# pyani-plus/pyani-plus

Measured on AMD Instinct MI355X. Metric: pairwise genome comparisons/sec (N x N ANI matrix), higher is better.
Workload: dtype u64

## Files before the change

### pyani_plus_amd/csrc/kmer_hash.hip

```cpp
#include <cstdlib>
#include <type_traits>
#include <utility>

#include "pa_internal.h"
#include "murmur_dev.h"

namespace {

using namespace pa_dev;

constexpr int kThreads = 256;
constexpr uint32_t kStageCap = 1024;
constexpr uint32_t kStageCapSecond = 512;

constexpr int pow2_floor(int k) { int c = 1; while (2 * c <= k) c *= 2; return c; }

__device__ __forceinline__ uint32_t find_genome(const uint32_t *__restrict__ genome_blk, uint32_t n, uint32_t blk) {
  uint32_t lo = 0, hi = n;
  while (hi - lo > 1) {
    uint32_t mid = (lo + hi) >> 1;
    if (genome_blk[mid] <= blk) lo = mid; else hi = mid;
  }
  return lo;
}

__device__ __forceinline__ void region_append(const CandSink &s, uint32_t g, uint64_t h) {
  const uint64_t slot = atomicAdd(&s.cursor[g], 1u);
  if (slot < s.region_off[g + 1] - s.region_off[g]) s.cand_hash[s.region_off[g] + slot] = h; else *s.overflow = 1u;
}

__device__ __forceinline__ void append_candidate(const CandSink &s, uint32_t g, uint64_t h) {
  if (s.region_off) {
    region_append(s, g, h);
  } else {
    const unsigned long long slot = atomicAdd(reinterpret_cast<unsigned long long *>(s.count), 1ULL);
    if (slot < s.cap) {
      s.cand_hash[slot] = h;
      s.cand_genome[slot] = g;
    }
  }
}

template <uint32_t Cap>
__device__ __forceinline__ void stage_candidate(const CandSink &s, uint64_t (&s_hash)[Cap], uint32_t (&s_blk)[Cap],
                                                uint32_t &s_n, uint32_t t, uint64_t h) {
  const uint32_t slot = atomicAdd(&s_n, 1u);
  if (slot < Cap) {
    s_hash[slot] = h;
    s_blk[slot] = t;
  } else if (s.region_off) {
    region_append(s, find_genome(s.genome_blk, s.n_genomes, t), h);
  } else {
    const unsigned long long g = atomicAdd(reinterpret_cast<unsigned long long *>(s.count), 1ULL);
    if (g < s.cap) {
      s.cand_hash[g] = h;
      s.cand_genome[g] = find_genome(s.genome_blk, s.n_genomes, t);
    }
  }
}

template <uint32_t Cap>
__device__ __forceinline__ void flush_staged(const CandSink &s, const uint64_t (&s_hash)[Cap], const uint32_t (&s_blk)[Cap],
                                             const uint32_t &s_n, unsigned long long &s_base, uint32_t blk0, uint32_t n_blocks64) {
  const uint32_t tid = threadIdx.x;
  __syncthreads();
  const uint32_t n = min(s_n, Cap);
  if (n == 0) return;
  if (s.region_off) {
    const uint32_t b0 = blk0 + blockIdx.x * kThreads;
    const uint32_t b1 = min(b0 + (uint32_t)kThreads, n_blocks64) - 1u;
    const uint32_t g0 = find_genome(s.genome_blk, s.n_genomes, b0);
    if (s.genome_blk[g0 + 1] > b1) {
      if (tid == 0) s_base = atomicAdd(&s.cursor[g0], n);
      __syncthreads();
      const uint64_t room = s.region_off[g0 + 1] - s.region_off[g0];
      uint64_t *__restrict__ dst = s.cand_hash + s.region_off[g0];
      for (uint32_t i = tid; i < n; i += kThreads) {
        const uint64_t slot = s_base + i;
        if (slot < room) dst[slot] = s_hash[i]; else *s.overflow = 1u;
      }
    } else {
      for (uint32_t i = tid; i < n; i += kThreads)
        region_append(s, find_genome(s.genome_blk, s.n_genomes, s_blk[i]), s_hash[i]);
    }
    return;
  }
  if (tid == 0) s_base = atomicAdd(reinterpret_cast<unsigned long long *>(s.count), (unsigned long long)n);
  __syncthreads();
  const unsigned long long base = s_base;
  for (uint32_t i = tid; i < n; i += kThreads) {
    const unsigned long long g = base + i;
    if (g < s.cap) {
      s.cand_hash[g] = s_hash[i];
      s.cand_genome[g] = find_genome(s.genome_blk, s.n_genomes, s_blk[i]);
    }
  }
}

__device__ __forceinline__ uint32_t rev_groups32(uint32_t x) {
  x = __builtin_bitreverse32(x);
  return ((x >> 1) & 0x55555555u) | ((x & 0x55555555u) << 1);
}

enum WordForm { kArithmetic = 0, kFirstTables = 1, kSecondTables = 2 };
template <int K, WordForm FORM>
__global__ __launch_bounds__(kThreads) void kmer_hash_kernel(
    const uint4 *__restrict__ packed, const uint2 *__restrict__ mask, const uint64_t *__restrict__ dirty, uint32_t n_blocks64,
    const uint32_t *__restrict__ genome_blk, uint32_t n_genomes, uint64_t max_hash,
    uint64_t *__restrict__ cand_hash, uint32_t *__restrict__ cand_genome, uint64_t cap,
    unsigned long long *__restrict__ count, const uint64_t *__restrict__ region_off, uint32_t *__restrict__ cursor,
    uint32_t *__restrict__ overflow, uint32_t blk0) {
  static_assert(K >= 1 && K <= 32, "a k-mer is one 64-bit register pair");
  constexpr uint32_t kCap = FORM == kSecondTables ? kStageCapSecond : kStageCap;
  __shared__ uint64_t s_hash[kCap];
  __shared__ uint32_t s_blk[kCap];
  __shared__ uint32_t s_n;
  __shared__ unsigned long long s_base;
  constexpr int kWords = (K + 7) / 8;
  __shared__ uint64_t s_lo[FORM == kFirstTables ? kWords : 1][256];
  __shared__ uint4 s_w[FORM == kSecondTables ? kWords : 1][256];
  __shared__ uint32_t s_hi[FORM != kArithmetic ? kWords : 1][256];

  const uint32_t tid = threadIdx.x;
  const CandSink sink{cand_hash, cand_genome, cap, reinterpret_cast<uint64_t *>(count), region_off, cursor, overflow, genome_blk, n_genomes};
  const uint32_t max_hi = (uint32_t)(max_hash >> 32);
  const bool take_all = max_hi == 0xffffffffu;
  const uint32_t screen_hi = max_hi + 1u;
  if (tid == 0) s_n = 0;
  if constexpr (FORM == kFirstTables) fill_first_products(s_lo, s_hi, tid, std::integral_constant<int, K>{});
  if constexpr (FORM == kSecondTables) fill_second_products(s_w, s_hi, tid, K);
  __syncthreads();

  const uint32_t t = blk0 + blockIdx.x * kThreads + tid;
  if (t < n_blocks64) {
    const uint4 cur = packed[t];
    uint2 pw = make_uint2(0u, 0u);
    if (t > 0) pw = reinterpret_cast<const uint2 *>(packed)[2 * (uint64_t)t - 1];
    uint32_t d1 = 0u, d2 = 0u;
    const uint32_t wave_blk = __builtin_amdgcn_readfirstlane(t & ~63u);
    const uint64_t dirty_word = dirty[wave_blk >> 6];
    if ((dirty_word >> (t & 63u)) & 1ull) {
      const uint2 m = mask[t];
      uint32_t d0 = t > 0 ? mask[t - 1].y : 0xffffffffu;
      d1 = m.x;
      d2 = m.y;
      int c = 1;
#pragma unroll
      for (; 2 * c <= K; c *= 2) {
        d2 |= alignbit(d2, d1, 32 - c);
        d1 |= alignbit(d1, d0, 32 - c);
        d0 |= d0 << c;
      }
      constexpr int cc = pow2_floor(K);
      constexpr int r = K - cc;
      if constexpr (r > 0) {
        d2 |= alignbit(d2, d1, 32 - r);
        d1 |= alignbit(d1, d0, 32 - r);
      }
    }
    const uint32_t bad[2] = {d1, d2};
    if ((d1 & d2) != 0xffffffffu) {
      constexpr uint64_t kMask = (K == 32) ? ~0ULL : ((1ULL << (2 * K)) - 1);
      constexpr uint32_t kMaskHi = (uint32_t)(kMask >> 32);
      uint32_t fw[8] = {pw.x, pw.y, cur.x, cur.y, cur.z, cur.w, 0u, 0u};
      uint32_t rw[6];
#pragma unroll
      for (int j = 0; j < 6; ++j) rw[j] = ~rev_groups32(fw[5 - j]);
      auto columns = [&](auto base_tag, int i_begin, int i_end) {
        constexpr int kBase = decltype(base_tag)::value;
#pragma unroll 1
        for (int i = i_begin; i < i_end; ++i) {
          constexpr int kOff = 33 - K;
          const uint32_t fo = 2u * (uint32_t)((i + kOff) & 15), ro = 30u - 2u * (uint32_t)i;
          uint32_t A[5], B[5];
#pragma unroll
          for (int j = 0; j < 5; ++j) {
            A[j] = alignbit(fw[kBase + j + 1], fw[kBase + j], fo);
            B[j] = alignbit(rw[j + 1], rw[j], ro);
          }
#pragma unroll
          for (int wi = 0; wi < 4; ++wi) {
            const uint32_t f_lo = A[wi], f_hi = A[wi + 1], r_lo = B[3 - wi], r_hi = B[4 - wi];
          const uint64_t f_lsb = u64_of(f_lo, f_hi) & kMask, r_lsb = u64_of(r_lo, r_hi) & kMask;
          const uint64_t fwd = __builtin_amdgcn_uicmpl(f_lsb, r_lsb, 37 );
          uint32_t clo, chi;
          asm("s_nop 1\n\tv_cndmask_b32_e64 %0, %1, %2, %3" : "=v"(clo) : "v"((uint32_t)r_lsb), "v"((uint32_t)f_lsb), "s"(fwd));
          asm("v_cndmask_b32_e64 %0, %1, %2, %3" : "=v"(chi) : "v"((uint32_t)(r_lsb >> 32)), "v"((uint32_t)(f_lsb >> 32)), "s"(fwd), "v"(clo));
          uint64_t P[4] = {0, 0, 0, 0};
#pragma unroll
          for (int j = 0; j < kWords; ++j) {
            const uint32_t src = j < 2 ? clo : chi;
            if constexpr (FORM == kSecondTables) {
              P[j] = second_product(s_w, s_hi, j, src);
            } else if constexpr (FORM == kFirstTables) {
              P[j] = first_product(s_lo, s_hi, j, src);
            } else {
              const uint32_t glo = (src >> (16 * (j & 1))) & 0xffu, ghi = (src >> (16 * (j & 1) + 8)) & 0xffu;
              const uint64_t word = u64_of(ascii_group(glo, K - 8 * j), ascii_group(ghi, K - 8 * j - 4));
              P[j] = word * ((j & 1) ? kC2 : kC1);
            }
          }
          (void)kMaskHi;
          uint64_t U, V;
          if constexpr (FORM == kSecondTables) murmur3_pre_last_mul_of_seconds<K>(P, U, V); else murmur3_pre_last_mul<K>(P, U, V);
          if (passes_screen(U, V, take_all, screen_hi)) {
            const uint64_t h = last_mul_and_fold(U, V);
            if (h > max_hash || ((bad[wi >> 1] >> (16 * (wi & 1) + i)) & 1u)) continue;
            stage_candidate(sink, s_hash, s_blk, s_n, t, h);
          }
          }
        }
      };
      constexpr int kOff0 = 33 - K, kSplit = (kOff0 & 15) ? 16 - (kOff0 & 15) : 16;
      columns(std::integral_constant<int, (kOff0 >> 4)>{}, 0, kSplit);
      if constexpr (kSplit < 16) columns(std::integral_constant<int, (kOff0 >> 4) + 1>{}, kSplit, 16);
    }
  }
  flush_staged(sink, s_hash, s_blk, s_n, s_base, blk0, n_blocks64);
}

template <int K>
__global__ __launch_bounds__(kThreads) void kmer_hash_wide_kernel(
    const uint4 *__restrict__ packed, const uint2 *__restrict__ mask, const uint64_t *__restrict__ dirty, uint32_t n_blocks64,
    const uint32_t *__restrict__ genome_blk, uint32_t n_genomes, uint64_t max_hash,
    uint64_t *__restrict__ cand_hash, uint32_t *__restrict__ cand_genome, uint64_t cap,
    unsigned long long *__restrict__ count, const uint64_t *__restrict__ region_off, uint32_t *__restrict__ cursor,
    uint32_t *__restrict__ overflow, uint32_t blk0) {
  static_assert(K >= 33 && K <= 64, "k-mers of 65 to 128 bits");
  __shared__ uint64_t s_hash[kStageCap];
  __shared__ uint32_t s_blk[kStageCap];
  __shared__ uint32_t s_n;
  __shared__ unsigned long long s_base;
  constexpr int kWords = (K + 7) / 8;
  __shared__ uint64_t s_lo[kWords][256];
  __shared__ uint32_t s_hi[kWords][256];
  const uint32_t tid = threadIdx.x;
  const CandSink sink{cand_hash, cand_genome, cap, reinterpret_cast<uint64_t *>(count), region_off, cursor, overflow, genome_blk, n_genomes};
  const uint32_t max_hi = (uint32_t)(max_hash >> 32);
  const bool take_all = max_hi == 0xffffffffu;
  const uint32_t screen_hi = max_hi + 1u;
  if (tid == 0) s_n = 0;
  fill_first_products(s_lo, s_hi, tid, std::integral_constant<int, K>{});
  __syncthreads();

  const uint32_t t = blk0 + blockIdx.x * kThreads + tid;
  if (t < n_blocks64) {
    const uint4 cur = packed[t];
    const uint4 prev = t > 0 ? packed[t - 1] : make_uint4(0u, 0u, 0u, 0u);
    uint32_t d2 = 0u, d3 = 0u;
    const uint32_t wave_blk = __builtin_amdgcn_readfirstlane(t & ~63u);
    const uint64_t dirty_word = dirty[wave_blk >> 6];
    const uint64_t before = wave_blk ? dirty[(wave_blk >> 6) - 1] >> 63 : 1ull;
    const uint64_t dirty_or_prev = dirty_word | (dirty_word << 1) | before;
    if ((dirty_or_prev >> (t & 63u)) & 1ull) {
      const uint2 m = mask[t];
      uint32_t d0 = 0xffffffffu, d1 = 0xffffffffu;
      if (t > 0) { const uint2 mp = mask[t - 1]; d0 = mp.x; d1 = mp.y; }
      d2 = m.x;
      d3 = m.y;
#pragma unroll
      for (int c = 1; c <= 16; c *= 2) {
        d3 |= alignbit(d3, d2, 32 - c);
        d2 |= alignbit(d2, d1, 32 - c);
        d1 |= alignbit(d1, d0, 32 - c);
        d0 |= d0 << c;
      }
      if constexpr (K == 64) {
        d3 |= d2; d2 |= d1; d1 |= d0;
      } else {
        constexpr int r = K - 32;
        d3 |= alignbit(d3, d2, 32 - r);
        d2 |= alignbit(d2, d1, 32 - r);
        d1 |= alignbit(d1, d0, 32 - r);
      }
    }
    const uint32_t bad[2] = {d2, d3};
    if ((d2 & d3) != 0xffffffffu) {
      constexpr uint32_t kMask2 = (2 * K - 64 >= 32) ? 0xffffffffu : ((1u << (2 * K - 64)) - 1u);
      constexpr uint32_t kMask3 = (2 * K - 96 >= 32) ? 0xffffffffu : (2 * K - 96 <= 0 ? 0u : ((1u << ((2 * K - 96) & 31)) - 1u));
      const uint32_t fw[10] = {prev.x, prev.y, prev.z, prev.w, cur.x, cur.y, cur.z, cur.w, 0u, 0u};
      uint32_t rw[10];
#pragma unroll
      for (int j = 0; j < 10; ++j) rw[j] = ~rev_groups32(fw[9 - j]);
      auto columns = [&](auto base_tag, int i_begin, int i_end) {
        constexpr int kBase = decltype(base_tag)::value;
#pragma unroll 1
        for (int i = i_begin; i < i_end; ++i) {
          constexpr int kOff = 65 - K;
          const uint32_t fo = 2u * (uint32_t)((i + kOff) & 15), ro = 30u - 2u * (uint32_t)i;
          uint32_t A[7], B[7];
#pragma unroll
          for (int j = 0; j < 7; ++j) {
            A[j] = alignbit(fw[kBase + j + 1], fw[kBase + j], fo);
            B[j] = alignbit(rw[j + 3], rw[j + 2], ro);
          }
#pragma unroll
          for (int wi = 0; wi < 4; ++wi) {
            const uint32_t f0 = A[wi], f1 = A[wi + 1], f2 = A[wi + 2] & kMask2, f3 = A[wi + 3] & kMask3;
            const uint32_t r0 = B[3 - wi], r1 = B[4 - wi], r2 = B[5 - wi] & kMask2, r3 = B[6 - wi] & kMask3;
            const uint64_t lt_hi = __builtin_amdgcn_uicmpl(u64_of(f2, f3), u64_of(r2, r3), 36 );
            const uint64_t eq_hi = __builtin_amdgcn_uicmpl(u64_of(f2, f3), u64_of(r2, r3), 32 );
            const uint64_t le_lo = __builtin_amdgcn_uicmpl(u64_of(f0, f1), u64_of(r0, r1), 37 );
            const uint64_t fwd = lt_hi | (eq_hi & le_lo);
            uint32_t c0, c1, c2, c3;
            asm("s_nop 1\n\tv_cndmask_b32_e64 %0, %1, %2, %3" : "=v"(c0) : "v"(r0), "v"(f0), "s"(fwd));
            asm("v_cndmask_b32_e64 %0, %1, %2, %3" : "=v"(c1) : "v"(r1), "v"(f1), "s"(fwd), "v"(c0));
            asm("v_cndmask_b32_e64 %0, %1, %2, %3" : "=v"(c2) : "v"(r2), "v"(f2), "s"(fwd), "v"(c1));
            asm("v_cndmask_b32_e64 %0, %1, %2, %3" : "=v"(c3) : "v"(r3), "v"(f3), "s"(fwd), "v"(c2));
            const uint32_t cw[4] = {c0, c1, c2, c3};
            uint64_t P[8] = {0, 0, 0, 0, 0, 0, 0, 0};
#pragma unroll
            for (int j = 0; j < kWords; ++j) P[j] = first_product(s_lo, s_hi, j, cw[j >> 1]);
            uint64_t U, V;
            murmur3_pre_last_mul<K>(P, U, V);
            if (passes_screen(U, V, take_all, screen_hi)) {
              const uint64_t h = last_mul_and_fold(U, V);
              if (h > max_hash || ((bad[wi >> 1] >> (16 * (wi & 1) + i)) & 1u)) continue;
              stage_candidate(sink, s_hash, s_blk, s_n, t, h);
            }
          }
        }
      };
      constexpr int kOff0 = 65 - K, kSplit = (kOff0 & 15) ? 16 - (kOff0 & 15) : 16;
      columns(std::integral_constant<int, (kOff0 >> 4)>{}, 0, kSplit);
      if constexpr (kSplit < 16) columns(std::integral_constant<int, (kOff0 >> 4) + 1>{}, kSplit, 16);
    }
  }
  flush_staged(sink, s_hash, s_blk, s_n, s_base, blk0, n_blocks64);
}

constexpr int kLongIter = 32;
__global__ __launch_bounds__(kThreads) void kmer_hash_long_kernel(
    const uint32_t *__restrict__ packed, const uint32_t *__restrict__ mask, uint64_t pos0, uint64_t pos1, uint32_t k,
    const uint32_t *__restrict__ genome_blk, uint32_t n_genomes, uint64_t max_hash, uint64_t *__restrict__ cand_hash,
    uint32_t *__restrict__ cand_genome, uint64_t cap, unsigned long long *__restrict__ count,
    const uint64_t *__restrict__ region_off, uint32_t *__restrict__ cursor, uint32_t *__restrict__ overflow) {
  __shared__ uint64_t s_lo[8][256];
  __shared__ uint32_t s_hi[8][256];
  const uint32_t tid = threadIdx.x;
  const CandSink sink{cand_hash, cand_genome, cap, reinterpret_cast<uint64_t *>(count), region_off, cursor, overflow, genome_blk, n_genomes};
  const uint32_t n_words = (k + 7u) >> 3;
  const uint32_t max_hi = (uint32_t)(max_hash >> 32);
  const bool take_all = max_hi == 0xffffffffu;
  const uint32_t screen_hi = max_hi + 1u;
  fill_first_products(s_lo, s_hi, tid, k);
  __syncthreads();
  const uint64_t wg_first = pos0 + ((uint64_t)blockIdx.y * gridDim.x + blockIdx.x) * (uint64_t)(kThreads * kLongIter);
#pragma unroll 1
  for (int it = 0; it < kLongIter; ++it) {
  const uint64_t e = wg_first + (uint64_t)it * kThreads + tid;
  if (e >= pos1 || e + 1 < k) continue;
  const uint64_t a = e + 1 - k;
  {
    const uint64_t m0 = a >> 5, m_last = e >> 5;
    const uint32_t sm = (uint32_t)(a & 31u);
    const uint32_t w0 = mask[m0], w1 = m0 + 1 <= m_last ? mask[m0 + 1] : 0u, w2 = m0 + 2 <= m_last ? mask[m0 + 2] : 0u;
    const uint32_t b0 = alignbit(w1, w0, sm), b1 = alignbit(w2, w1, sm);
    const uint32_t top = k == 64 ? 0xffffffffu : ((1u << (k - 32u)) - 1u);
    if (b0 | (b1 & top)) continue;
  }
  uint32_t F[4], R[4];
  {
    const uint64_t p0 = a >> 4, p_last = e >> 4;
    const uint32_t sp = 2u * (uint32_t)(a & 15u);
    uint32_t w[5];
#pragma unroll
    for (int i = 0; i < 5; ++i) w[i] = p0 + i <= p_last ? packed[p0 + i] : 0u;
#pragma unroll
    for (int i = 0; i < 4; ++i) F[i] = alignbit(w[i + 1], w[i], sp);
    const uint32_t used = 2u * k - 64u;
    if (used < 32u) { F[2] &= (1u << used) - 1u; F[3] = 0u; }
    else if (used < 64u) F[3] &= (1u << (used - 32u)) - 1u;
    const uint32_t C[6] = {~rev_groups32(F[3]), ~rev_groups32(F[2]), ~rev_groups32(F[1]), ~rev_groups32(F[0]), 0u, 0u};
    const uint32_t s = 128u - 2u * k, ws = s >> 5, bs = s & 31u;
#pragma unroll
    for (int i = 0; i < 4; ++i) R[i] = ws ? alignbit(C[i + 2], C[i + 1], bs) : alignbit(C[i + 1], C[i], bs);
    if (used < 32u) { R[2] &= (1u << used) - 1u; R[3] = 0u; }
    else if (used < 64u) R[3] &= (1u << (used - 32u)) - 1u;
  }
  const uint64_t f_hi = u64_of(F[2], F[3]), f_lo = u64_of(F[0], F[1]), r_hi = u64_of(R[2], R[3]), r_lo = u64_of(R[0], R[1]);
  const bool fwd = f_hi < r_hi || (f_hi == r_hi && f_lo <= r_lo);
  uint32_t c[4];
#pragma unroll
  for (int i = 0; i < 4; ++i) c[i] = fwd ? F[i] : R[i];
  uint64_t P[8] = {0, 0, 0, 0, 0, 0, 0, 0};
#pragma unroll
  for (uint32_t j = 0; j < 8; ++j) {
    if (j >= n_words) break;
    P[j] = first_product(s_lo, s_hi, j, c[j >> 1]);
  }
  uint64_t U, V;
  murmur3_pre_last_mul_rt(P, k, U, V);
  if (!passes_screen(U, V, take_all, screen_hi)) continue;
  const uint64_t h = last_mul_and_fold(U, V);
  if (h > max_hash) continue;
  append_candidate(sink, find_genome(genome_blk, n_genomes, (uint32_t)(e >> 6)), h);
  }
}

template <class Kernel>
int launch_blocks(pa_ctx *c, const char *name, Kernel kernel, const KmerHashArgs &a) {
  const ArenaView &v = a.arena;
  const CandSink &s = a.sink;
  return pa_launch(c, name, kernel, false, ceil_div(v.n_blocks64 - a.blk0, kThreads), kThreads, 0, a.stream,
                   reinterpret_cast<const uint4 *>(v.packed), reinterpret_cast<const uint2 *>(v.mask), v.dirty,
                   (uint32_t)v.n_blocks64, s.genome_blk, s.n_genomes, a.max_hash, s.cand_hash, s.cand_genome, s.cap,
                   reinterpret_cast<unsigned long long *>(s.count), s.region_off, s.cursor, s.overflow, (uint32_t)a.blk0);
}

template <int K>
int launch_k(pa_ctx *c, const KmerHashArgs &a) {
  if constexpr (K > 32) {
    return launch_blocks(c, "kmer_hash_wide_kernel", kmer_hash_wide_kernel<K>, a);
  } else {
#ifdef PA_TOOLS
    if constexpr (K == 31) {
      const char *v = PA_TOOL_ENV("PA_KMER_VARIANT");
      if (v && v[0] == '0') return launch_blocks(c, "kmer_hash_kernel<31, kArithmetic>", kmer_hash_kernel<K, kArithmetic>, a);
      if (v && v[0] == '1') return launch_blocks(c, "kmer_hash_kernel<31, kFirstTables>", kmer_hash_kernel<K, kFirstTables>, a);
    }
#endif
    return launch_blocks(c, "kmer_hash_kernel", kmer_hash_kernel<K, kSecondTables>, a);
  }
}

}

int pa_launch_kmer_hash(pa_ctx *c, const KmerHashArgs &a) {
  const uint64_t n_blocks64 = a.arena.n_blocks64;
  PA_REQUIRE(n_blocks64 < (1ULL << 32), "arena too large: %llu blocks of 64 bases", (unsigned long long)n_blocks64);
  if (n_blocks64 <= a.blk0) return PA_OK;
  const char *long_form = PA_TOOL_ENV("PA_KMER_LONG");
  if (a.k > 32 && a.k <= 64 && long_form && long_form[0] == 'p') {
    const CandSink &s = a.sink;
    const uint64_t pos0 = a.blk0 * 64, pos1 = n_blocks64 * 64;
    const uint64_t per_wg = (uint64_t)kThreads * kLongIter;
    const uint64_t n_wg = (pos1 - pos0 + per_wg - 1) / per_wg;
    const uint32_t gx = (uint32_t)std::min<uint64_t>(n_wg, 1u << 20), gy = (uint32_t)((n_wg + gx - 1) / gx);
    PA_REQUIRE(gy <= 65535u, "arena too large for one launch of the long k-mer kernel: %llu positions", (unsigned long long)(pos1 - pos0));
    return PA_LAUNCH_ON(c, a.stream, kmer_hash_long_kernel, LaunchDim(gx, gy), kThreads, 0, a.arena.packed, a.arena.mask, pos0, pos1, a.k,
                        s.genome_blk, s.n_genomes, a.max_hash, s.cand_hash, s.cand_genome, s.cap,
                        reinterpret_cast<unsigned long long *>(s.count), s.region_off, s.cursor, s.overflow);
  }
  PA_REQUIRE((a.blk0 & 63u) == 0, "k-mer hash launch must start at a multiple of 64 blocks, not %llu", (unsigned long long)a.blk0);
  int status = PA_E_INVALID;
  if (!dispatch_value(a.k, value_list<1, 64>{}, [&](auto k) { status = launch_k<k()>(c, a); })) pa_set_error("k=%u outside [1,64]", a.k);
  return status;
}
```

### pyani_plus_amd/csrc/murmur_dev.h

```cpp
#pragma once

#include <hip/hip_runtime.h>

#include <cstdint>

#include "murmur_words.h"

namespace pa_dev {

__device__ __forceinline__ uint32_t alignbit(uint32_t hi, uint32_t lo, uint32_t sh) {
  return __builtin_amdgcn_alignbit(hi, lo, sh);
}

__device__ __forceinline__ uint64_t u64_of(uint32_t lo, uint32_t hi) { return ((uint64_t)hi << 32) | lo; }

__device__ __forceinline__ uint64_t rotl64(uint64_t x, int r) {
  const uint32_t lo = (uint32_t)x, hi = (uint32_t)(x >> 32);
  if (r == 32) return u64_of(hi, lo);
  if (r < 32) return u64_of(alignbit(lo, hi, 32 - r), alignbit(hi, lo, 32 - r));
  return u64_of(alignbit(hi, lo, 64 - r), alignbit(lo, hi, 64 - r));
}

__device__ __forceinline__ uint64_t fmix64(uint64_t k) {
  k ^= k >> 33;
  k *= 0xff51afd7ed558ccdULL;
  k ^= k >> 33;
  k *= 0xc4ceb9fe1a85ec53ULL;
  k ^= k >> 33;
  return k;
}


__device__ __forceinline__ uint64_t times5_plus(uint64_t h, uint64_t c) {
  uint64_t t;
  asm("v_lshl_add_u64 %0, %1, 2, %1" : "=v"(t) : "v"(h));
  return t + c;
}

constexpr uint64_t kF1 = 0xff51afd7ed558ccdULL, kF2 = 0xc4ceb9fe1a85ec53ULL;

template <int K, int N>
__device__ __forceinline__ void murmur3_pre_last_mul(const uint64_t (&P)[N], uint64_t &U, uint64_t &V) {
  static_assert(N >= (K + 7) / 8, "one first product per 8-byte word of the k-mer");
  uint64_t h1 = 42, h2 = 42;
  constexpr int nblocks = K / 16;
  constexpr int tail = K % 16;
#pragma unroll
  for (int i = 0; i < nblocks; ++i) {
    const uint64_t k1 = rotl64(P[2 * i], 31) * kC2;
    h1 ^= k1;
    if (i == 0) {
      h1 = times5_plus(rotl64(h1, 27), 5ULL * 42ULL + 0x52dce729ULL);
    } else {
      h1 = rotl64(h1, 27) + h2;
      h1 = times5_plus(h1, 0x52dce729ULL);
    }
    const uint64_t k2 = rotl64(P[2 * i + 1], 33) * kC1;
    h2 ^= k2;
    h2 = rotl64(h2, 31) + h1;
    h2 = times5_plus(h2, 0x38495ab5ULL);
  }
  if constexpr (tail > 8) h2 ^= rotl64(P[2 * nblocks + 1], 33) * kC1;
  if constexpr (tail > 0) h1 ^= rotl64(P[2 * nblocks], 31) * kC2;
  h1 ^= (uint64_t)K; h2 ^= (uint64_t)K;
  h1 += h2; h2 += h1;
  h1 ^= h1 >> 33; h1 *= kF1; h1 ^= h1 >> 33;
  h2 ^= h2 >> 33; h2 *= kF1; h2 ^= h2 >> 33;
  U = h1;
  V = h2;
}

template <int K, int N>
__device__ __forceinline__ void murmur3_pre_last_mul_of_seconds(const uint64_t (&Kw)[N], uint64_t &U, uint64_t &V) {
  static_assert(N >= (K + 7) / 8, "one second product per 8-byte word of the k-mer");
  uint64_t h1 = 42, h2 = 42;
  constexpr int nblocks = K / 16;
  constexpr int tail = K % 16;
#pragma unroll
  for (int i = 0; i < nblocks; ++i) {
    h1 ^= Kw[2 * i];
    if (i == 0) {
      h1 = times5_plus(rotl64(h1, 27), 5ULL * 42ULL + 0x52dce729ULL);
    } else {
      h1 = rotl64(h1, 27) + h2;
      h1 = times5_plus(h1, 0x52dce729ULL);
    }
    h2 ^= Kw[2 * i + 1];
    uint64_t r2 = rotl64(h2, 31);
    asm("" : "+v"(r2));
    h2 = times5_plus(r2 + h1, 0x38495ab5ULL);
  }
  if constexpr (tail > 8) h2 ^= Kw[2 * nblocks + 1];
  if constexpr (tail > 0) h1 ^= Kw[2 * nblocks];
  h1 ^= (uint64_t)K; h2 ^= (uint64_t)K;
  h1 += h2; h2 += h1;
  h1 ^= h1 >> 33; h1 *= kF1; h1 ^= h1 >> 33;
  h2 ^= h2 >> 33; h2 *= kF1; h2 ^= h2 >> 33;
  U = h1;
  V = h2;
}

__device__ __forceinline__ void murmur3_pre_last_mul_rt(const uint64_t (&P)[8], uint32_t k, uint64_t &U, uint64_t &V) {
  uint64_t h1 = 42, h2 = 42;
  const uint32_t nblocks = k >> 4, tail = k & 15u;
#pragma unroll
  for (uint32_t i = 0; i < 4; ++i) {
    if (i >= nblocks) break;
    h1 ^= rotl64(P[2 * i], 31) * kC2;
    h1 = rotl64(h1, 27) + h2;
    h1 = times5_plus(h1, 0x52dce729ULL);
    h2 ^= rotl64(P[2 * i + 1], 33) * kC1;
    h2 = rotl64(h2, 31) + h1;
    h2 = times5_plus(h2, 0x38495ab5ULL);
  }
  uint64_t t1 = 0, t2 = 0;
#pragma unroll
  for (uint32_t i = 0; i < 4; ++i)
    if (i == nblocks) { t1 = P[2 * i]; t2 = P[2 * i + 1]; }
  if (tail > 8) h2 ^= rotl64(t2, 33) * kC1;
  if (tail > 0) h1 ^= rotl64(t1, 31) * kC2;
  h1 ^= (uint64_t)k;
  h2 ^= (uint64_t)k;
  h1 += h2;
  h2 += h1;
  h1 ^= h1 >> 33; h1 *= kF1; h1 ^= h1 >> 33;
  h2 ^= h2 >> 33; h2 *= kF1; h2 ^= h2 >> 33;
  U = h1;
  V = h2;
}

__device__ __forceinline__ uint32_t last_mul_high_sum_plus1(uint64_t U, uint64_t V) {
  constexpr uint32_t c0 = (uint32_t)kF2, c1 = (uint32_t)(kF2 >> 32);
  const uint32_t u0 = (uint32_t)U, u1 = (uint32_t)(U >> 32), v0 = (uint32_t)V, v1 = (uint32_t)(V >> 32);
  return (__umulhi(u0, c0) + __umulhi(v0, c0) + 1u) + ((u0 + v0) * c1 + (u1 + v1) * c0);
}

__device__ __forceinline__ bool passes_screen(uint64_t U, uint64_t V, bool take_all, uint32_t screen_hi) {
  return take_all || last_mul_high_sum_plus1(U, V) <= screen_hi;
}
__device__ __forceinline__ uint64_t last_mul_and_fold(uint64_t U, uint64_t V) {
  const uint64_t X = U * kF2, Y = V * kF2;
  return (X ^ (X >> 33)) + (Y ^ (Y >> 33));
}

template <int K, int N>
__device__ __forceinline__ uint64_t murmur3_from_products(const uint64_t (&P)[N]) {
  uint64_t U, V;
  murmur3_pre_last_mul<K, N>(P, U, V);
  return last_mul_and_fold(U, V);
}

template <int W, class KInt>
__device__ __forceinline__ void fill_first_products(uint64_t (&s_lo)[W][256], uint32_t (&s_hi)[W][256], uint32_t tid, KInt k_) {
  const int k = (int)k_;
  const int n_words = (int)(((uint32_t)k + 7u) >> 3);
#pragma unroll
  for (int j = 0; j < n_words; ++j) {
    const uint64_t cj = (j & 1) ? kC2 : kC1;
    s_lo[j][tid] = (uint64_t)ascii_group(tid, k - 8 * j) * cj;
    s_hi[j][tid] = (uint32_t)((uint64_t)ascii_group(tid, k - 8 * j - 4) * cj);
  }
}

template <int W>
__device__ __forceinline__ uint64_t first_product(const uint64_t (&s_lo)[W][256], const uint32_t (&s_hi)[W][256], uint32_t j, uint32_t src) {
  const uint32_t glo = (src >> (16u * (j & 1u))) & 0xffu, ghi = (src >> (16u * (j & 1u) + 8u)) & 0xffu;
  const uint64_t lo = s_lo[j][glo];
  return u64_of((uint32_t)lo, (uint32_t)(lo >> 32) + s_hi[j][ghi]);
}

template <int W>
__device__ __forceinline__ void fill_second_products(uint4 (&s_w)[W][256], uint32_t (&s_b)[W][256], uint32_t tid, int k) {
#pragma unroll
  for (int j = 0; j < W; ++j) {
    const WordLoEntry e = word_lo_entry(j, k, tid);
    s_w[j][tid] = make_uint4(e.t_lo, e.t_hi, e.a_hi, e.pad);
    s_b[j][tid] = word_hi_entry(j, k, tid);
  }
}

template <uint32_t SH>
__device__ __forceinline__ uint32_t byte_offset(uint32_t src, uint32_t byte) {
  uint32_t r;
  const uint32_t sh = SH;
  switch (byte) {
    case 0: asm("v_lshlrev_b32_sdwa %0, %1, %2 dst_sel:DWORD dst_unused:UNUSED_PAD src0_sel:DWORD src1_sel:BYTE_0" : "=v"(r) : "v"(sh), "v"(src)); break;
    case 1: asm("v_lshlrev_b32_sdwa %0, %1, %2 dst_sel:DWORD dst_unused:UNUSED_PAD src0_sel:DWORD src1_sel:BYTE_1" : "=v"(r) : "v"(sh), "v"(src)); break;
    case 2: asm("v_lshlrev_b32_sdwa %0, %1, %2 dst_sel:DWORD dst_unused:UNUSED_PAD src0_sel:DWORD src1_sel:BYTE_2" : "=v"(r) : "v"(sh), "v"(src)); break;
    default: asm("v_lshlrev_b32_sdwa %0, %1, %2 dst_sel:DWORD dst_unused:UNUSED_PAD src0_sel:DWORD src1_sel:BYTE_3" : "=v"(r) : "v"(sh), "v"(src)); break;
  }
  return r;
}

template <int W>
__device__ __forceinline__ uint64_t second_product(const uint4 (&s_w)[W][256], const uint32_t (&s_b)[W][256], int j, uint32_t src) {
  const uint32_t off_w = byte_offset<4>(src, 2u * (j & 1)), off_b = byte_offset<2>(src, 2u * (j & 1) + 1u);
  typedef uint32_t u32x4 __attribute__((ext_vector_type(4)));
  u32x4 e = *reinterpret_cast<const u32x4 *>(reinterpret_cast<const char *>(&s_w[j][0]) + off_w);
  asm("" : "+v"(e));
  const uint32_t b = *reinterpret_cast<const uint32_t *>(reinterpret_cast<const char *>(&s_b[j][0]) + off_b);
  return second_product_of(j, e.x, e.y, e.z, b);
}

}
```

### pyani_plus_amd/csrc/murmur_words.h

```cpp
#pragma once

#include <cstdint>

#if defined(__HIPCC__)
#include <hip/hip_runtime.h>
#define PA_WORDS_FN __host__ __device__ __forceinline__
#else
#define PA_WORDS_FN inline
#endif

namespace pa_dev {

constexpr uint64_t kC1 = 0x87c37b91114253d5ULL, kC2 = 0x4cf5ad432745937fULL;

PA_WORDS_FN uint32_t ascii4(uint32_t b8) {
#if defined(__HIP_DEVICE_COMPILE__)
  uint32_t u = (b8 | (b8 << 12)) & 0x000F000Fu;
  uint32_t v = (u | (u << 6)) & 0x03030303u;
  return __builtin_amdgcn_perm(0u, 0x54474341u, v);
#else
  uint32_t a = 0;
  for (int i = 0; i < 4; ++i) a |= ((0x54474341u >> (8 * ((b8 >> (2 * i)) & 3u))) & 0xffu) << (8 * i);
  return a;
#endif
}

PA_WORDS_FN uint32_t ascii_group(uint32_t b8, int nv) {
  const uint32_t a = ascii4(b8);
  return nv >= 4 ? a : (nv <= 0 ? 0u : (a & ((1u << (8 * nv)) - 1u)));
}

PA_WORDS_FN constexpr uint64_t word_c_first(int j) { return (j & 1) ? kC2 : kC1; }
PA_WORDS_FN constexpr uint64_t word_c_second(int j) { return (j & 1) ? kC1 : kC2; }

struct WordLoEntry {
  uint32_t t_lo, t_hi, a_hi, pad;
};

PA_WORDS_FN WordLoEntry word_lo_entry(int j, int k, uint32_t g) {
  const uint64_t a = (uint64_t)ascii_group(g, k - 8 * j) * word_c_first(j);
  const uint32_t a_lo = (uint32_t)a;
  const uint64_t cb = word_c_second(j);
  const uint64_t t = (j & 1) ? (((uint64_t)a_lo << 33) + (a_lo >> 31)) * cb : ((uint64_t)a_lo << 31) * cb;
  return WordLoEntry{(uint32_t)t, (uint32_t)(t >> 32), (uint32_t)(a >> 32), 0u};
}

PA_WORDS_FN uint32_t word_hi_entry(int j, int k, uint32_t g) {
  return (uint32_t)((uint64_t)ascii_group(g, k - 8 * j - 4) * word_c_first(j));
}

PA_WORDS_FN uint64_t second_product_of(int j, uint32_t t_lo, uint32_t t_hi, uint32_t a_hi, uint32_t b) {
  const uint32_t s = a_hi + b;
  const uint64_t t = ((uint64_t)t_hi << 32) | t_lo;
  if (j & 1) {
    const uint64_t c = word_c_second(j) << 1;
    const uint64_t m = (uint64_t)s * (uint32_t)c + t;
    return ((uint64_t)((uint32_t)(m >> 32) + s * (uint32_t)(c >> 32)) << 32) | (uint32_t)m;
  }
  const uint64_t c = word_c_second(j);
  const uint32_t x = s >> 1;
  const uint64_t m = (uint64_t)x * (uint32_t)c + t;
  return ((uint64_t)((uint32_t)(m >> 32) + (x * (uint32_t)(c >> 32) + (s << 31))) << 32) | (uint32_t)m;
}

}
```

Before: 86.92 million.

## Process multiple tiles per workgroup and simplify the hash screen arithmetic

Each workgroup now loops over several 256-block tiles (default 4, overridable by env) instead of one. This amortises the per-workgroup shared-memory table fill and synchronisation. When the expected candidate count fits, staged candidates are flushed once per group rather than per tile. The pre-screen now computes one high-word estimate from U+V instead of two separate mulhi terms, with a looser bound and threshold. This cuts ALU work per k-mer but may let slightly more candidates through to the full fold.

```diff
diff --git a/pyani_plus_amd/csrc/kmer_hash.hip b/pyani_plus_amd/csrc/kmer_hash.hip
--- a/pyani_plus_amd/csrc/kmer_hash.hip
+++ b/pyani_plus_amd/csrc/kmer_hash.hip
@@ -61,14 +61,12 @@
 
 template <uint32_t Cap>
 __device__ __forceinline__ void flush_staged(const CandSink &s, const uint64_t (&s_hash)[Cap], const uint32_t (&s_blk)[Cap],
-                                             const uint32_t &s_n, unsigned long long &s_base, uint32_t blk0, uint32_t n_blocks64) {
+                                             const uint32_t &s_n, unsigned long long &s_base, uint32_t b0, uint32_t b1) {
   const uint32_t tid = threadIdx.x;
   __syncthreads();
   const uint32_t n = min(s_n, Cap);
   if (n == 0) return;
   if (s.region_off) {
-    const uint32_t b0 = blk0 + blockIdx.x * kThreads;
-    const uint32_t b1 = min(b0 + (uint32_t)kThreads, n_blocks64) - 1u;
     const uint32_t g0 = find_genome(s.genome_blk, s.n_genomes, b0);
     if (s.genome_blk[g0 + 1] > b1) {
       if (tid == 0) s_base = atomicAdd(&s.cursor[g0], n);
@@ -97,6 +95,31 @@
   }
 }
 
+constexpr uint32_t kTilesPerGroup = 4;
+
+template <uint32_t Cap, class Tile>
+__device__ __forceinline__ void for_each_tile(const CandSink &s, uint64_t (&s_hash)[Cap], uint32_t (&s_blk)[Cap], uint32_t &s_n,
+                                              unsigned long long &s_base, uint32_t blk0, uint32_t n_blocks64, uint32_t tiles,
+                                              uint64_t max_hash, Tile &&tile) {
+  const uint32_t tid = threadIdx.x;
+  const uint32_t first = blk0 + blockIdx.x * (kThreads * tiles);
+  const uint32_t n_here = min((uint32_t)kThreads * tiles, n_blocks64 - first);
+  const bool flush_once = ((((max_hash >> 32) + 1u) * (uint64_t)(64u * kThreads * tiles)) >> 32) <= Cap / 2;
+#pragma unroll 1
+  for (uint32_t off = 0; off < n_here; off += kThreads) {
+    if (off + tid < n_here) tile(first + off + tid);
+    if (!flush_once) {
+      flush_staged(s, s_hash, s_blk, s_n, s_base, first + off, first + min(off + (uint32_t)kThreads, n_here) - 1u);
+      if (off + kThreads < n_here) {
+        __syncthreads();
+        if (tid == 0) s_n = 0;
+        __syncthreads();
+      }
+    }
+  }
+  if (flush_once) flush_staged(s, s_hash, s_blk, s_n, s_base, first, first + n_here - 1u);
+}
+
 __device__ __forceinline__ uint32_t rev_groups32(uint32_t x) {
   x = __builtin_bitreverse32(x);
   return ((x >> 1) & 0x55555555u) | ((x & 0x55555555u) << 1);
@@ -109,7 +132,7 @@
     const uint32_t *__restrict__ genome_blk, uint32_t n_genomes, uint64_t max_hash,
     uint64_t *__restrict__ cand_hash, uint32_t *__restrict__ cand_genome, uint64_t cap,
     unsigned long long *__restrict__ count, const uint64_t *__restrict__ region_off, uint32_t *__restrict__ cursor,
-    uint32_t *__restrict__ overflow, uint32_t blk0) {
+    uint32_t *__restrict__ overflow, uint32_t blk0, uint32_t tiles) {
   static_assert(K >= 1 && K <= 32, "a k-mer is one 64-bit register pair");
   constexpr uint32_t kCap = FORM == kSecondTables ? kStageCapSecond : kStageCap;
   __shared__ uint64_t s_hash[kCap];
@@ -124,15 +147,14 @@
   const uint32_t tid = threadIdx.x;
   const CandSink sink{cand_hash, cand_genome, cap, reinterpret_cast<uint64_t *>(count), region_off, cursor, overflow, genome_blk, n_genomes};
   const uint32_t max_hi = (uint32_t)(max_hash >> 32);
-  const bool take_all = max_hi == 0xffffffffu;
-  const uint32_t screen_hi = max_hi + 1u;
+  const bool take_all = screen_takes_all(max_hi);
+  const uint32_t screen_hi = screen_bound(max_hi);
   if (tid == 0) s_n = 0;
   if constexpr (FORM == kFirstTables) fill_first_products(s_lo, s_hi, tid, std::integral_constant<int, K>{});
   if constexpr (FORM == kSecondTables) fill_second_products(s_w, s_hi, tid, K);
   __syncthreads();
 
-  const uint32_t t = blk0 + blockIdx.x * kThreads + tid;
-  if (t < n_blocks64) {
+  for_each_tile(sink, s_hash, s_blk, s_n, s_base, blk0, n_blocks64, tiles, max_hash, [&](const uint32_t t) {
     const uint4 cur = packed[t];
     uint2 pw = make_uint2(0u, 0u);
     if (t > 0) pw = reinterpret_cast<const uint2 *>(packed)[2 * (uint64_t)t - 1];
@@ -215,8 +237,7 @@
       columns(std::integral_constant<int, (kOff0 >> 4)>{}, 0, kSplit);
       if constexpr (kSplit < 16) columns(std::integral_constant<int, (kOff0 >> 4) + 1>{}, kSplit, 16);
     }
-  }
-  flush_staged(sink, s_hash, s_blk, s_n, s_base, blk0, n_blocks64);
+  });
 }
 
 template <int K>
@@ -225,7 +246,7 @@
     const uint32_t *__restrict__ genome_blk, uint32_t n_genomes, uint64_t max_hash,
     uint64_t *__restrict__ cand_hash, uint32_t *__restrict__ cand_genome, uint64_t cap,
     unsigned long long *__restrict__ count, const uint64_t *__restrict__ region_off, uint32_t *__restrict__ cursor,
-    uint32_t *__restrict__ overflow, uint32_t blk0) {
+    uint32_t *__restrict__ overflow, uint32_t blk0, uint32_t tiles) {
   static_assert(K >= 33 && K <= 64, "k-mers of 65 to 128 bits");
   __shared__ uint64_t s_hash[kStageCap];
   __shared__ uint32_t s_blk[kStageCap];
@@ -237,14 +258,13 @@
   const uint32_t tid = threadIdx.x;
   const CandSink sink{cand_hash, cand_genome, cap, reinterpret_cast<uint64_t *>(count), region_off, cursor, overflow, genome_blk, n_genomes};
   const uint32_t max_hi = (uint32_t)(max_hash >> 32);
-  const bool take_all = max_hi == 0xffffffffu;
-  const uint32_t screen_hi = max_hi + 1u;
+  const bool take_all = screen_takes_all(max_hi);
+  const uint32_t screen_hi = screen_bound(max_hi);
   if (tid == 0) s_n = 0;
   fill_first_products(s_lo, s_hi, tid, std::integral_constant<int, K>{});
   __syncthreads();
 
-  const uint32_t t = blk0 + blockIdx.x * kThreads + tid;
-  if (t < n_blocks64) {
+  for_each_tile(sink, s_hash, s_blk, s_n, s_base, blk0, n_blocks64, tiles, max_hash, [&](const uint32_t t) {
     const uint4 cur = packed[t];
     const uint4 prev = t > 0 ? packed[t - 1] : make_uint4(0u, 0u, 0u, 0u);
     uint32_t d2 = 0u, d3 = 0u;
@@ -325,8 +345,7 @@
       columns(std::integral_constant<int, (kOff0 >> 4)>{}, 0, kSplit);
       if constexpr (kSplit < 16) columns(std::integral_constant<int, (kOff0 >> 4) + 1>{}, kSplit, 16);
     }
-  }
-  flush_staged(sink, s_hash, s_blk, s_n, s_base, blk0, n_blocks64);
+  });
 }
 
 constexpr int kLongIter = 32;
@@ -341,8 +360,8 @@
   const CandSink sink{cand_hash, cand_genome, cap, reinterpret_cast<uint64_t *>(count), region_off, cursor, overflow, genome_blk, n_genomes};
   const uint32_t n_words = (k + 7u) >> 3;
   const uint32_t max_hi = (uint32_t)(max_hash >> 32);
-  const bool take_all = max_hi == 0xffffffffu;
-  const uint32_t screen_hi = max_hi + 1u;
+  const bool take_all = screen_takes_all(max_hi);
+  const uint32_t screen_hi = screen_bound(max_hi);
   fill_first_products(s_lo, s_hi, tid, k);
   __syncthreads();
   const uint64_t wg_first = pos0 + ((uint64_t)blockIdx.y * gridDim.x + blockIdx.x) * (uint64_t)(kThreads * kLongIter);
@@ -402,10 +421,15 @@
 int launch_blocks(pa_ctx *c, const char *name, Kernel kernel, const KmerHashArgs &a) {
   const ArenaView &v = a.arena;
   const CandSink &s = a.sink;
-  return pa_launch(c, name, kernel, false, ceil_div(v.n_blocks64 - a.blk0, kThreads), kThreads, 0, a.stream,
+  uint32_t tiles = kTilesPerGroup;
+  if (const char *t = PA_TOOL_ENV("PA_KMER_TILES")) {
+    const unsigned long n = strtoul(t, nullptr, 10);
+    if (n >= 1 && n <= 64) tiles = (uint32_t)n;
+  }
+  return pa_launch(c, name, kernel, false, ceil_div(v.n_blocks64 - a.blk0, (uint64_t)kThreads * tiles), kThreads, 0, a.stream,
                    reinterpret_cast<const uint4 *>(v.packed), reinterpret_cast<const uint2 *>(v.mask), v.dirty,
                    (uint32_t)v.n_blocks64, s.genome_blk, s.n_genomes, a.max_hash, s.cand_hash, s.cand_genome, s.cap,
-                   reinterpret_cast<unsigned long long *>(s.count), s.region_off, s.cursor, s.overflow, (uint32_t)a.blk0);
+                   reinterpret_cast<unsigned long long *>(s.count), s.region_off, s.cursor, s.overflow, (uint32_t)a.blk0, tiles);
 }
 
 template <int K>
diff --git a/pyani_plus_amd/csrc/murmur_dev.h b/pyani_plus_amd/csrc/murmur_dev.h
--- a/pyani_plus_amd/csrc/murmur_dev.h
+++ b/pyani_plus_amd/csrc/murmur_dev.h
@@ -36,8 +36,6 @@
   asm("v_lshl_add_u64 %0, %1, 2, %1" : "=v"(t) : "v"(h));
   return t + c;
 }
-
-constexpr uint64_t kF1 = 0xff51afd7ed558ccdULL, kF2 = 0xc4ceb9fe1a85ec53ULL;
 
 template <int K, int N>
 __device__ __forceinline__ void murmur3_pre_last_mul(const uint64_t (&P)[N], uint64_t &U, uint64_t &V) {
@@ -129,18 +127,8 @@
   V = h2;
 }
 
-__device__ __forceinline__ uint32_t last_mul_high_sum_plus1(uint64_t U, uint64_t V) {
-  constexpr uint32_t c0 = (uint32_t)kF2, c1 = (uint32_t)(kF2 >> 32);
-  const uint32_t u0 = (uint32_t)U, u1 = (uint32_t)(U >> 32), v0 = (uint32_t)V, v1 = (uint32_t)(V >> 32);
-  return (__umulhi(u0, c0) + __umulhi(v0, c0) + 1u) + ((u0 + v0) * c1 + (u1 + v1) * c0);
-}
-
 __device__ __forceinline__ bool passes_screen(uint64_t U, uint64_t V, bool take_all, uint32_t screen_hi) {
-  return take_all || last_mul_high_sum_plus1(U, V) <= screen_hi;
-}
-__device__ __forceinline__ uint64_t last_mul_and_fold(uint64_t U, uint64_t V) {
-  const uint64_t X = U * kF2, Y = V * kF2;
-  return (X ^ (X >> 33)) + (Y ^ (Y >> 33));
+  return take_all || screen_word(U, V) <= screen_hi;
 }
 
 template <int K, int N>
diff --git a/pyani_plus_amd/csrc/murmur_words.h b/pyani_plus_amd/csrc/murmur_words.h
--- a/pyani_plus_amd/csrc/murmur_words.h
+++ b/pyani_plus_amd/csrc/murmur_words.h
@@ -63,4 +63,20 @@
   return ((uint64_t)((uint32_t)(m >> 32) + (x * (uint32_t)(c >> 32) + (s << 31))) << 32) | (uint32_t)m;
 }
 
+constexpr uint64_t kF1 = 0xff51afd7ed558ccdULL, kF2 = 0xc4ceb9fe1a85ec53ULL;
+
+PA_WORDS_FN uint64_t last_mul_and_fold(uint64_t U, uint64_t V) {
+  const uint64_t X = U * kF2, Y = V * kF2;
+  return (X ^ (X >> 33)) + (Y ^ (Y >> 33));
 }
+
+PA_WORDS_FN uint32_t screen_word(uint64_t U, uint64_t V) {
+  constexpr uint32_t c0 = (uint32_t)kF2, c1 = (uint32_t)(kF2 >> 32);
+  const uint64_t w = U + V;
+  const uint32_t w0 = (uint32_t)w, w1 = (uint32_t)(w >> 32);
+  return ((uint32_t)(((uint64_t)w0 * c0) >> 32) + 1u) + (w0 * c1 + w1 * c0);
+}
+PA_WORDS_FN constexpr bool screen_takes_all(uint32_t max_hi) { return max_hi >= 0xfffffffdu; }
+PA_WORDS_FN constexpr uint32_t screen_bound(uint32_t max_hi) { return max_hi + 2u; }
+
+}
```

Result: faster. 89.00 million, median of 6 (+2.4%).
